# CrystalAnalyst/Lsm

Measured on AMD Instinct MI355X. Metric: GiB/s device-resident SSTable block encode+decode, 4 KiB blocks, 1/2/4/8 GPU, higher is better.
Workload: dtype u8; 1 GPU; U: 1048576 blocks/GPU x block_size 4096, decode + re-encode (16-B uniform keys, 100-B values); blocks_per_gpu=1048576, entries_per_gpu=32474205, encoded_bytes_per_gpu=4226189427, decoded_bytes_per_gpu=4286595060, block_size=4096, segments_per_gpu=2045, parallelism=block-sharded x1 (no data-path collective), encode_output=segments packed (lsmblk_encode_batch), rccl_world=1

## Files before the change

lsm_amd/csrc/lsmblk_gpu.hip:

```cpp
#include "lsmblk_dev.hpp"

namespace {


struct DecodeArgs {
  const uint8_t* blocks;
  const uint64_t* blk_off;
  uint64_t nblk;
  uint8_t* keys;
  uint32_t* key_off;
  uint8_t* vals;
  uint32_t* val_off;
  uint64_t* ts;
  uint64_t entry_cap, key_cap, val_cap;
  uint64_t* stats;
  const uint32_t* agg;
  const uint64_t* tile_pre;
  uint32_t tail;
  uint64_t* blk_ent;
  uint32_t skip;
  uint64_t* bagg;
  uint64_t* bbase;
  uint64_t* tagg;
  uint64_t* tinc;
  uint64_t lag;
  uint64_t lag_bytes;
  uint64_t* dbg;
  uint32_t tag, poll;
};

constexpr uint32_t kTile = 64;
constexpr uint32_t kDbgTiles = 32768, kDbgWords = 16 + 8 * kDbgTiles;
__device__ __forceinline__ void dbg_trace(uint64_t* dbg, uint64_t t, uint32_t k) {
  if (kDiag && dbg && t < kDbgTiles && lane_id() == 0) dbg[16 + 8 * t + k] = __builtin_amdgcn_s_memrealtime();
}


constexpr uint32_t kLB = 2;
constexpr uint32_t kDecMB = 2;
#ifndef LSMBLK_XEB
#define LSMBLK_XEB 4
#endif
constexpr uint32_t kEB = LSMBLK_XEB;
constexpr uint32_t kEBBlock = 2;


constexpr uint32_t kDecImg = 4128;
constexpr uint32_t kDecMaxE = 128;
constexpr uint32_t kDecKeyImg = 2176;
constexpr uint32_t kDecMapN = 256;
constexpr uint32_t kDecOut = 4032;
static_assert(kDecOut <= 16 * kDecMapN && 16 * kDecMapN <= kDecImg, "the chunk map covers the value run");

struct alignas(16) DecLds {
  uint8_t img[kDecImg];
  alignas(16) uint8_t kimg[kDecKeyImg];
  alignas(16) uint16_t cmap[kDecMapN];
};
static_assert(sizeof(DecLds) <= (160 << 10) / 24, "decode LDS: room for 24 blocks per CU");

struct DecTables {
  uint16_t epos[kDecMaxE], pfx[kDecMaxE], sfx[kDecMaxE];
  uint32_t kout[kDecMaxE + 1], vout[kDecMaxE + 1];
};
static_assert(sizeof(DecTables) <= kDecImg, "large-block tables overlay the image");

struct DecEnt {
  uint32_t epos, p, s, kout, vout, vl;
};

__device__ __forceinline__ void lds_read16(const uint8_t* base, uint32_t x, uint32_t (&v)[4]) {
  const u32x4 q = *reinterpret_cast<const u32x4*>(base + x);
  v[0] = q.x, v[1] = q.y, v[2] = q.z, v[3] = q.w;
}

constexpr int kLdAux = 0;

template <class Img>
__device__ void dec_simple_outputs(const DecodeArgs& a, const Img& im, const BlockHdr& h,
                                   uint64_t E0, uint64_t K0, uint64_t V0) {
  const uint32_t l = lane_id();
  uint64_t kc = 0, vc = 0;
  for (uint32_t c = 0; c < h.n; c += 64) {
    const uint32_t k = c + l;
    uint32_t off = 0, p = 0, s = 0, vl = 0;
    if (k < h.n) parse_entry(im, h, k, off, p, s, vl);
    const uint64_t kl = p + s;
    const uint64_t ki = wave_incl_scan<uint64_t>(kl), vi = wave_incl_scan<uint64_t>(vl);
    const uint64_t kpos = K0 + kc + ki - kl, vpos = V0 + vc + vi - vl;
    kc += __shfl(ki, 63, 64);
    vc += __shfl(vi, 63, 64);
    if (k < h.n) {
      const uint64_t e = E0 + k;
      if (e < a.entry_cap) {
        a.ts[e] = im.u64(off + 4 + s);
        a.key_off[e] = uint32_t(kpos);
        a.val_off[e] = uint32_t(vpos);
      }
      for (uint32_t t = 0; t < p; ++t)
        if (kpos + t < a.key_cap) a.keys[kpos + t] = uint8_t(im.u8(4 + t));
      for (uint32_t t = 0; t < s; ++t)
        if (kpos + p + t < a.key_cap) a.keys[kpos + p + t] = uint8_t(im.u8(off + 4 + t));
      for (uint32_t t = 0; t < vl; ++t)
        if (vpos + t < a.val_cap) a.vals[vpos + t] = uint8_t(im.u8(off + 14 + s + t));
    }
  }
}

__device__ __forceinline__ void st16(const rsrc_t& R, uint32_t off, const uint32_t (&v)[4]) {
  const u32x4 q = {v[0], v[1], v[2], v[3]};
  __builtin_amdgcn_raw_buffer_store_b128(q, R, off, 0, 0);
}

__device__ __forceinline__ void st_short(const rsrc_t& R, uint32_t off, uint32_t len, const uint32_t (&v)[4]) {
  if (len >= 8) {
    __builtin_amdgcn_raw_buffer_store_b64(u32x2{v[0], v[1]}, R, off, 0, 0);
    const uint32_t x = len - 8, sh = x & 3;
    const uint32_t w0 = x < 4 ? v[0] : v[1], w1 = x < 4 ? v[1] : v[2], w2 = x < 4 ? v[2] : v[3];
    __builtin_amdgcn_raw_buffer_store_b64(
        u32x2{__builtin_amdgcn_alignbyte(w1, w0, sh), __builtin_amdgcn_alignbyte(w2, w1, sh)}, R, off + x, 0, 0);
  } else if (len >= 4) {
    __builtin_amdgcn_raw_buffer_store_b32(v[0], R, off, 0, 0);
    __builtin_amdgcn_raw_buffer_store_b32(__builtin_amdgcn_alignbyte(v[1], v[0], len - 4), R, off + len - 4, 0, 0);
  } else {
    for (uint32_t i = 0; i < len; ++i)
      __builtin_amdgcn_raw_buffer_store_b8(uint8_t(v[0] >> (8 * i)), R, off + i, 0, 0);
  }
}

__device__ __forceinline__ void lds_st_short(uint8_t* p, uint32_t len, const uint32_t (&v)[4]) {
  if (len >= 8) {
    const uint32_t x = len - 8, sh = x & 3;
    const uint32_t w0 = x < 4 ? v[0] : v[1], w1 = x < 4 ? v[1] : v[2], w2 = x < 4 ? v[2] : v[3];
    *reinterpret_cast<u32x2*>(p) = u32x2{v[0], v[1]};
    *reinterpret_cast<u32x2*>(p + x) = u32x2{__builtin_amdgcn_alignbyte(w1, w0, sh), __builtin_amdgcn_alignbyte(w2, w1, sh)};
  } else if (len >= 4) {
    *reinterpret_cast<uint32_t*>(p) = v[0];
    *reinterpret_cast<uint32_t*>(p + len - 4) = __builtin_amdgcn_alignbyte(v[1], v[0], len - 4);
  } else {
    for (uint32_t i = 0; i < len; ++i) p[i] = uint8_t(v[0] >> (8 * i));
  }
}

struct GlbSink {
  rsrc_t RK, RV;
  uint32_t kb, vb;
  __device__ __forceinline__ void put16(bool val, uint32_t off, const uint32_t (&v)[4]) const {
    st16(val ? RV : RK, (val ? vb : kb) + off, v);
  }
  __device__ __forceinline__ void put_short(bool val, uint32_t off, uint32_t len, const uint32_t (&v)[4]) const {
    st_short(val ? RV : RK, (val ? vb : kb) + off, len, v);
  }
};
struct LdsSink {
  uint8_t* kimg;
  uint32_t kb;
  uint16_t* cmap;
  uint32_t vb;
  __device__ __forceinline__ void put16(bool, uint32_t off, const uint32_t (&v)[4]) const {
    *reinterpret_cast<u32x4*>(kimg + kb + off) = u32x4{v[0], v[1], v[2], v[3]};
  }
  __device__ __forceinline__ void put_short(bool, uint32_t off, uint32_t len, const uint32_t (&v)[4]) const {
    lds_st_short(kimg + kb + off, len, v);
  }
};

template <class Sink>
__device__ __forceinline__ void dec_entry_runs(const DecodeArgs& a, DecLds& L, uint32_t lead, uint32_t n,
                                               const DecEnt (&ent)[2], uint64_t E0, uint64_t K0, uint64_t V0,
                                               const Sink& out, uint32_t skip, uint32_t (&eh)[2][4],
                                               uint32_t (&et)[2][4]) {
  const uint32_t l = lane_id();
  const uint8_t* img = L.img;
  const uint32_t fk = lead + 4;
#pragma unroll
  for (uint32_t it = 0; it < 2; ++it) {
    if (64 * it >= n) break;
    const uint32_t k = 64 * it + l;
    const bool live = k < n;
    const uint32_t epos = ent[it].epos, p = ent[it].p, s = ent[it].s;
    const uint32_t kout = ent[it].kout, vout = ent[it].vout, vl = ent[it].vl;
    const uint32_t sb = lead + epos + 4;
    const uint32_t kl = p + s;
    const bool kirr = live && (kl < 16 || sb < p);
    const bool kuni = !__ballot(kirr);
    const uint32_t nkmax = __builtin_amdgcn_readlane(wave_incl_max32(live ? (kl + 15) >> 4 : 0u), 63);
    uint32_t nvmax = 0;
    if constexpr (!std::is_same_v<Sink, LdsSink>)
      nvmax = __builtin_amdgcn_readlane(wave_incl_max32(live && vl >= 16 ? (vl + 15) >> 4 : 0u), 63);
    if (!live) continue;
    if (!(skip & 8)) {
      const uint64_t e = E0 + k;
      const u32x2 q = LSMBLK_XALIGNED_LDS ? lds_qw_al(img, sb + s) : *reinterpret_cast<const u32x2*>(img + sb + s);
      a.ts[e] = __builtin_bswap64((uint64_t(q.y) << 32) | q.x);
      a.key_off[e] = uint32_t(K0 + kout);
      a.val_off[e] = uint32_t(V0 + vout);
    }
    if (!(skip & 2)) {
      auto merged = [&](uint32_t o, uint32_t (&v)[4]) {
        const u32x4 sq = *reinterpret_cast<const u32x4*>(img + sb + o - p);
        const u32x4 fq = *reinterpret_cast<const u32x4*>(img + fk + o);
        const uint32_t sv[4] = {sq.x, sq.y, sq.z, sq.w}, fv[4] = {fq.x, fq.y, fq.z, fq.w};
#pragma unroll
        for (uint32_t d = 0; d < 4; ++d) {
          const int32_t nf = int32_t(p) - int32_t(o + 4 * d);
          const uint32_t m = nf <= 0 ? 0u : nf >= 4 ? ~0u : (1u << (8 * nf)) - 1;
          v[d] = (fv[d] & m) | (sv[d] & ~m);
        }
      };
      if (kuni) {
        for (uint32_t t = 0; t < nkmax; ++t) {
          const uint32_t o = min(16 * t, kl - 16);
          uint32_t v[4];
          merged(o, v);
          out.put16(false, kout + o, v);
        }
      } else {
        for (uint32_t t = 0; t < kl; t += 16) {
          const uint32_t o = kl >= 16 ? min(t, kl - 16) : 0u;
          uint32_t v[4];
          if (sb + o >= p) {
            merged(o, v);
          } else {
#pragma unroll
            for (uint32_t d = 0; d < 4; ++d) {
              uint32_t wd = 0;
              for (uint32_t i = 0; i < 4; ++i) {
                const uint32_t x = o + 4 * d + i;
                wd |= uint32_t(x < p ? img[fk + x] : img[sb + x - p]) << (8 * i);
              }
              v[d] = wd;
            }
          }
          if (kl >= 16) out.put16(false, kout + o, v);
          else out.put_short(false, kout, kl, v);
        }
      }
    }
    const uint32_t src = sb + s + 10;
    if constexpr (std::is_same_v<Sink, LdsSink>) {
      if (vl && !(skip & 4)) {
        lds_read16(img, src, eh[it]);
        lds_read16(img, src + (vl > 16 ? vl - 16 : 0u), et[it]);
        const uint32_t vD = out.vb + vout;
        const uint32_t d = src - vD;
        for (uint32_t c = (vD + 15) >> 4; 16 * c + 16 <= vD + vl; ++c) out.cmap[c] = uint16_t(d + 16 * c);
      }
    } else if (!(skip & 4)) {
      if (vl >= 16) {
        for (uint32_t i0 = 0; i0 < nvmax; i0 += kLB) {
          u32x4 q[kLB];
          uint32_t o[kLB];
          const uint32_t am = (skip & 32) ? 15u : (skip & 64) ? 3u : 0u;
#pragma unroll
          for (uint32_t j = 0; j < kLB; ++j) {
            o[j] = min(16 * (i0 + j), vl - 16);
            q[j] = *reinterpret_cast<const u32x4*>(img + ((src + o[j]) & ~am));
          }
#pragma unroll
          for (uint32_t j = 0; j < kLB; ++j) {
            const uint32_t v[4] = {q[j].x, q[j].y, q[j].z, q[j].w};
            const uint32_t xa = (out.vb + vout + o[j]) & ~am;
            out.put16(true, xa >= out.vb ? xa - out.vb : xa + am + 1 - out.vb, v);
          }
        }
      } else if (vl) {
        const u32x4 q = *reinterpret_cast<const u32x4*>(img + src);
        const uint32_t v[4] = {q.x, q.y, q.z, q.w};
        out.put_short(true, vout, vl, v);
      }
    }
  }
}

template <uint32_t B = kLB>
__device__ __forceinline__ void flush_run(uint8_t* gdst_aligned, const uint8_t* lds, uint32_t lo, uint32_t len) {
  flush_chunks<B, LSMBLK_XDEC_STORE>(gdst_aligned, lds, lo, len, lane_id(), 64);
}

template <uint32_t B>
__device__ __forceinline__ void flush_run_masked(uint8_t* gdst_aligned, const uint8_t* lds, uint32_t lo, uint32_t len) {
  const uint32_t end = lo + len, nc = (end + 15) >> 4;
  const uint32_t l = lane_id();
  for (uint32_t c0 = 0; c0 < nc; c0 += 64 * B) {
    u32x4 q[B];
#pragma unroll
    for (uint32_t j = 0; j < B; ++j) {
      const uint32_t c = c0 + 64 * j + l;
      if (c < nc) q[j] = *reinterpret_cast<const u32x4*>(lds + 16 * c);
    }
#pragma unroll
    for (uint32_t j = 0; j < B; ++j) {
      const uint32_t c = c0 + 64 * j + l;
      if (c < nc) {
        const uint32_t v[4] = {q[j].x, q[j].y, q[j].z, q[j].w};
        const uint32_t a0 = 16 * c < lo ? lo - 16 * c : 0u;
        const uint32_t a1 = min(end - 16 * c, 16u);
        store_chunk(gdst_aligned + 16 * c, v, a0, a1);
      }
    }
  }
}

__device__ void dec_fast_outputs(const DecodeArgs& a, DecLds& L, uint32_t lead, const BlockHdr& h,
                                 const DecEnt (&ent)[2], uint64_t E0, uint64_t K0, uint64_t V0, uint32_t K,
                                 uint32_t V, uint32_t skip) {
  const uint32_t l = lane_id();
  const uint32_t n = h.n;
  const uint32_t kb = uint32_t(K0 & 15), vb = uint32_t(V0 & 15);
  int32_t dprev = 0;
  bool mono = true;
#pragma unroll
  for (uint32_t it = 0; it < 2; ++it) {
    if (64 * it >= n) break;
    const bool live = 64 * it + l < n;
    const int32_t d = live ? int32_t(lead + ent[it].epos + 14 + ent[it].s) - int32_t(vb + ent[it].vout) : 0x7FFFFFFF;
    const int32_t up = __shfl_up(d, 1, 64);
    mono = mono && d >= (l ? up : dprev);
    dprev = __builtin_amdgcn_readlane(d, 63);
  }
  const uint32_t krun = (kb + K + 15) & ~15u;
  if (!__ballot(!mono) && krun <= kDecKeyImg && krun + ((vb + V + 15) & ~15u) <= kDecOut) {
    static_assert(sizeof(DecLds::cmap) == 32 * 16, "the map is zeroed by 32 lanes");
    if (l < 32) reinterpret_cast<u32x4*>(L.cmap)[l] = u32x4{0, 0, 0, 0};
    wave_sync();
    uint32_t eh[2][4] = {}, et[2][4] = {};
    dec_entry_runs(a, L, lead, n, ent, E0, K0, V0, LdsSink{L.kimg, kb, L.cmap, vb}, skip, eh, et);
    wave_sync();
    flush_run(a.keys + (K0 - kb), L.kimg, kb, K);
    if (!(skip & 4)) {
      const uint32_t nw = (vb + V) >> 4;
      for (uint32_t c0 = 0; c0 < nw; c0 += 64 * kDecMB) {
        uint32_t src[kDecMB] = {};
        u32x4 v[kDecMB] = {};
#pragma unroll
        for (uint32_t j = 0; j < kDecMB; ++j) {
          const uint32_t c = c0 + 64 * j + l;
          src[j] = c < nw ? L.cmap[c] : 0u;
        }
#pragma unroll
        for (uint32_t j = 0; j < kDecMB; ++j)
          if (src[j]) v[j] = *reinterpret_cast<const u32x4*>(L.img + src[j]);
#pragma unroll
        for (uint32_t j = 0; j < kDecMB; ++j)
          if (src[j]) *reinterpret_cast<u32x4*>(L.img + 16 * (c0 + 64 * j + l)) = v[j];
      }
      wave_sync();
#pragma unroll
      for (uint32_t it = 0; it < 2; ++it) {
        if (64 * it >= n) break;
        const uint32_t vl = ent[it].vl;
        uint8_t* const o = L.img + vb + ent[it].vout;
        if (64 * it + l >= n) continue;
        if (vl >= 16) {
          *reinterpret_cast<u32x4*>(o) = u32x4{eh[it][0], eh[it][1], eh[it][2], eh[it][3]};
          *reinterpret_cast<u32x4*>(o + vl - 16) = u32x4{et[it][0], et[it][1], et[it][2], et[it][3]};
        } else if (vl) {
          lds_st_short(o, vl, eh[it]);
        }
      }
      wave_sync();
      flush_run(a.vals + (V0 - vb), L.img, vb, V);
    }
  } else {
    const GlbSink g{make_rsrc_exact(a.keys + (K0 - kb), kb + K), make_rsrc_exact(a.vals + (V0 - vb), vb + V), kb, vb};
    uint32_t eh[2][4], et[2][4];
    dec_entry_runs(a, L, lead, n, ent, E0, K0, V0, g, skip, eh, et);
  }
}

constexpr uint32_t kBigB = 8;

__device__ __forceinline__ u32x4 gload16(const rsrc_t& R, uint32_t off) {
  return __builtin_amdgcn_raw_buffer_load_b128(R, off, 0, 0);
}

__device__ __forceinline__ void copy_run(const rsrc_t& RS, uint32_t so, uint32_t lim, const rsrc_t& RD, uint32_t dof,
                                         uint32_t len) {
  if (len == 0) return;
  if (len < 16) {
    uint32_t v[4] = {0, 0, 0, 0};
    if (so + 16 <= lim) {
      const u32x4 q = gload16(RS, so);
      v[0] = q.x, v[1] = q.y, v[2] = q.z, v[3] = q.w;
    } else {
      for (uint32_t i = 0; i < len; ++i) v[i >> 2] |= __builtin_amdgcn_raw_buffer_load_b8(RS, so + i, 0, 0) << (8 * (i & 3));
    }
    st_short(RD, dof, len, v);
    return;
  }
  const uint32_t np = (len + 15) >> 4, last = len - 16;
  for (uint32_t j0 = 0; j0 < np; j0 += kBigB) {
    u32x4 q[kBigB];
#pragma unroll
    for (uint32_t j = 0; j < kBigB; ++j)
      if (j0 + j < np) q[j] = gload16(RS, so + min(16 * (j0 + j), last));
#pragma unroll
    for (uint32_t j = 0; j < kBigB; ++j)
      if (j0 + j < np) {
        const uint32_t v[4] = {q[j].x, q[j].y, q[j].z, q[j].w};
        st16(RD, dof + min(16 * (j0 + j), last), v);
      }
  }
}

__device__ __forceinline__ void copy_run1(const rsrc_t& RS, uint32_t so, uint32_t lim, const rsrc_t& RD, uint32_t dof,
                                          uint32_t len) {
  if (len < 16) {
    copy_run(RS, so, lim, RD, dof, len);
    return;
  }
  const uint32_t last = len - 16;
  for (uint32_t o = 0;; o += 16) {
    const uint32_t x = min(o, last);
    const u32x4 q = gload16(RS, so + x);
    const uint32_t v[4] = {q.x, q.y, q.z, q.w};
    st16(RD, dof + x, v);
    if (x == last) break;
  }
}

constexpr uint32_t kCoop = 16;
__device__ __forceinline__ void copy_run_wave(const rsrc_t& RS, uint32_t so, const rsrc_t& RD, uint32_t dof,
                                              uint32_t len) {
  const uint32_t l = lane_id();
  const uint32_t np = (len + 15) >> 4, last = len - 16;
  for (uint32_t j0 = 0; j0 < np; j0 += 64 * kBigB) {
    u32x4 q[kBigB];
#pragma unroll
    for (uint32_t j = 0; j < kBigB; ++j) {
      const uint32_t idx = j0 + 64 * j + l;
      if (idx < np) q[j] = gload16(RS, so + min(16 * idx, last));
    }
#pragma unroll
    for (uint32_t j = 0; j < kBigB; ++j) {
      const uint32_t idx = j0 + 64 * j + l;
      if (idx < np) {
        const uint32_t v[4] = {q[j].x, q[j].y, q[j].z, q[j].w};
        st16(RD, dof + min(16 * idx, last), v);
      }
    }
  }
}

constexpr uint32_t kCopyScratch = 4 * 64 + 64;
static_assert(4 * kCopyScratch <= kDecKeyImg, "the decode's large-block path lends its key image");

template <uint32_t B>
struct CopyBatch {
  u32x4 q[B];
  uint32_t dst[B];
};

template <uint32_t B, bool PIN = false>
__device__ __forceinline__ void copy_issue(const rsrc_t& RS, uint32_t g0, uint32_t total, uint32_t np, uint32_t first,
                                           uint32_t* sc, uint32_t& carry, CopyBatch<B>& c) {
  const uint32_t l = lane_id();
  if constexpr (PIN) {
#pragma unroll
    for (uint32_t j = 0; j < B; ++j) asm volatile("" : "=v"(c.q[j]));
  }
  const u32x4* rec = reinterpret_cast<const u32x4*>(sc);
  uint32_t* mark = sc + 4 * 64;
  uint32_t own[B];
#pragma unroll
  for (uint32_t j = 0; j < B; ++j) {
    const uint32_t G = g0 + 64 * j;
    own[j] = 0;
    if (G < total) {
      mark[l] = 0;
      wave_sync();
      if (np != 0 && first - G < 64u) mark[first - G] = l + 1;
      wave_sync();
      const uint32_t m = max(wave_incl_max32(mark[l]), carry);
      carry = __builtin_amdgcn_readlane(m, 63);
      own[j] = m - 1;
      wave_sync();
    }
  }
#pragma unroll
  for (uint32_t j = 0; j < B; ++j) {
    const uint32_t g = g0 + 64 * j + l;
    c.dst[j] = ~0u;
    if (g < total) {
      const u32x4 r = rec[own[j]];
      const uint32_t off = min(16 * (g - r.w), r.z);
      const uint32_t src = r.x + off;
      if constexpr (PIN) {
        if (j == 0) asm volatile("s_nop 4\n\tbuffer_load_dwordx4 %0, %1, %2, 0 offen" : "+v"(c.q[j]) : "v"(src), "s"(RS));
        else asm volatile("buffer_load_dwordx4 %0, %1, %2, 0 offen" : "+v"(c.q[j]) : "v"(src), "s"(RS));
      } else {
        c.q[j] = gload16(RS, src);
      }
      c.dst[j] = r.y + off;
    }
  }
}

template <uint32_t B>
__device__ __forceinline__ void copy_land(CopyBatch<B>& c) {
  asm volatile("s_waitcnt vmcnt(0)" ::: "memory");
#pragma unroll
  for (uint32_t j = 0; j < B; ++j) asm volatile("" : "+v"(c.q[j]));
}

template <uint32_t B>
__device__ __forceinline__ void copy_store(const rsrc_t& RD, const CopyBatch<B>& c) {
#pragma unroll
  for (uint32_t j = 0; j < B; ++j)
    if (c.dst[j] != ~0u) {
      const uint32_t v[4] = {c.q[j].x, c.q[j].y, c.q[j].z, c.q[j].w};
      st16(RD, c.dst[j], v);
    }
}

struct NoAfter {
  __device__ void operator()(uint32_t, uint32_t, uint32_t) const {}
};
template <uint32_t B = kBigB, bool PIN = false, class After = NoAfter>
__device__ __forceinline__ void copy_long_runs(bool longrun, const rsrc_t& RS, uint32_t so, const rsrc_t& RD,
                                               uint32_t dof, uint32_t len, uint32_t* sc, const After& after = After()) {
  const uint32_t l = lane_id();
  const uint32_t np = longrun ? (len + 15) >> 4 : 0u;
  const uint32_t incl = wave_incl_scan32(np);
  const uint32_t total = __builtin_amdgcn_readlane(incl, 63);
  const uint32_t first = incl - np;
  if (total == 0) {
    after(first, 0u, ~0u);
    return;
  }
  wave_sync();
  reinterpret_cast<u32x4*>(sc)[l] = u32x4{so, dof, len - 16, first};
  uint32_t carry = 0;
  for (uint32_t g0 = 0; g0 < total; g0 += 64 * B) {
    CopyBatch<B> c;
    copy_issue<B, PIN>(RS, g0, total, np, first, sc, carry, c);
    if constexpr (PIN) copy_land(c);
    copy_store(RD, c);
    after(first, g0, g0 + 64 * B >= total ? ~0u : g0 + 64 * B);
  }
}

__device__ __forceinline__ void dec_big_entry(const DecodeArgs& a, const DecTables& L, const GlbImg& im, uint32_t k,
                                              uint32_t lim, const rsrc_t& RK, uint32_t kb, uint64_t E0, uint64_t K0,
                                              uint64_t V0) {
  const rsrc_t& R = im.r;
  const uint32_t lead = im.lead, fk = lead + 4;
  const uint32_t epos = L.epos[k], p = L.pfx[k], s = L.sfx[k], kout = L.kout[k];
  const uint32_t sb = lead + epos + 4, kl = p + s;
  const uint64_t e = E0 + k;
  a.ts[e] = im.u64(epos + 4 + s);
  a.key_off[e] = uint32_t(K0 + kout);
  a.val_off[e] = uint32_t(V0 + L.vout[k]);
  for (uint32_t t = 0; t < kl; t += 16) {
    const uint32_t o = kl >= 16 ? min(t, kl - 16) : 0u;
    uint32_t v[4];
    if (sb + o >= p && sb + o - p + 16 <= lim && fk + o + 16 <= lim) {
      const u32x4 sq = gload16(R, sb + o - p), fq = gload16(R, fk + o);
      const uint32_t sv[4] = {sq.x, sq.y, sq.z, sq.w}, fv[4] = {fq.x, fq.y, fq.z, fq.w};
#pragma unroll
      for (uint32_t d = 0; d < 4; ++d) {
        const int32_t nf = int32_t(p) - int32_t(o + 4 * d);
        const uint32_t m = nf <= 0 ? 0u : nf >= 4 ? ~0u : (1u << (8 * nf)) - 1;
        v[d] = (fv[d] & m) | (sv[d] & ~m);
      }
    } else {
#pragma unroll
      for (uint32_t d = 0; d < 4; ++d) {
        uint32_t wd = 0;
        for (uint32_t i = 0; i < 4; ++i) {
          const uint32_t x = o + 4 * d + i;
          wd |= (x < p ? im.u8(4 + x) : im.u8(epos + 4 + x - p)) << (8 * i);
        }
        v[d] = wd;
      }
    }
    if (kl >= 16) st16(RK, kb + kout + o, v);
    else st_short(RK, kb + kout, kl, v);
  }
}

#ifndef LSMBLK_XDBB
#define LSMBLK_XDBB 8
#endif
constexpr uint32_t kDecBigB = LSMBLK_XDBB;

__device__ void dec_big_outputs(const DecodeArgs& a, const DecTables& L, const rsrc_t& R, uint32_t lead,
                                const BlockHdr& h, uint32_t n, uint64_t Eb, uint64_t K0, uint64_t V0, uint32_t K,
                                uint32_t V, uint32_t* sc) {
  const uint32_t l = lane_id();
  const uint32_t kb = uint32_t(K0 & 15), vb = uint32_t(V0 & 15);
  const rsrc_t RK = make_rsrc_exact(a.keys + (K0 - kb), kb + K), RV = make_rsrc_exact(a.vals + (V0 - vb), vb + V);
  const GlbImg im{R, lead};
  const uint32_t lim = lead + h.len;
  for (uint32_t c = 0; c < n; c += 64) {
    const uint32_t k = c + l;
    const bool live = k < n;
    uint32_t vsrc = 0, vdst = 0, vl = 0;
    if (live) {
      dec_big_entry(a, L, im, k, lim, RK, kb, Eb, K0, V0);
      vsrc = lead + L.epos[k] + 14 + L.sfx[k];
      vdst = vb + L.vout[k];
      vl = L.vout[k + 1] - L.vout[k];
      if (vl < kCoop) copy_run(R, vsrc, lim, RV, vdst, vl);
    }
    copy_long_runs<kDecBigB, true>(live && vl >= kCoop, R, vsrc, RV, vdst, vl, sc);
  }
}

template <bool lagm, class Mid, class Post, class PreWait>
__device__ void decode_block(const DecodeArgs& a, DecLds& L, uint64_t b, uint64_t start, uint64_t end, Mid&& mid,
                             Post&& post, PreWait&& pre_wait) {
  const uint32_t l = lane_id();
  uint32_t err = 0;
  const uint64_t tb = b / kTile, jb = b % kTile;
  uint32_t cn = 0, ck = 0, cv = 0;
  uint64_t tp0 = 0, tp1 = 0, tp2 = 0, gb = 0;
  if constexpr (!lagm) {
    if (l < jb) {
      const uint64_t q = tb * kTile + l;
      cn = a.agg[3 * q];
      ck = a.agg[3 * q + 1];
      cv = a.agg[3 * q + 2];
    }
    tp0 = a.tile_pre[3 * tb], tp1 = a.tile_pre[3 * tb + 1], tp2 = a.tile_pre[3 * tb + 2];
  }
  uint32_t len = 0;
  if (end < start + a.tail || end - start > 0x7FFFFFF0ull) err |= LSMBLK_ERR_MALFORMED;
  else len = uint32_t(end - start) - a.tail;
  const uint8_t* bp = a.blocks + start;
  const uint32_t lead = uni(uint32_t(reinterpret_cast<uintptr_t>(bp) & 15));
  const uint8_t* abase = bp - lead;
  const rsrc_t R = make_rsrc(abase, lead + len);
  const bool fits = lead + len + 15 <= kDecImg;

  BlockHdr h;
  if (fits) {
    const uint32_t nchunk = (lead + len + 15) >> 4;
    u32x4 v[5];
    if constexpr (lagm) {
      const uint32_t o = 16 * l, o4 = o + 4096;
      asm volatile(
          "s_nop 4\n\t"
          "buffer_load_dwordx4 %0, %5, %7, 0 offen\n\t"
          "buffer_load_dwordx4 %1, %5, %7, 0 offen offset:1024\n\t"
          "buffer_load_dwordx4 %2, %5, %7, 0 offen offset:2048\n\t"
          "buffer_load_dwordx4 %3, %5, %7, 0 offen offset:3072\n\t"
          "buffer_load_dwordx4 %4, %6, %7, 0 offen"
          : "=&v"(v[0]), "=&v"(v[1]), "=&v"(v[2]), "=&v"(v[3]), "=&v"(v[4])
          : "v"(o), "v"(o4), "s"(R));
      mid();
      asm volatile("s_waitcnt vmcnt(0)" ::: "memory");
#pragma unroll
      for (uint32_t i = 0; i < 5; ++i) asm volatile("" : "+v"(v[i]));
    } else {
#pragma unroll
      for (uint32_t i = 0; i < 5; ++i)
        v[i] = __builtin_amdgcn_raw_buffer_load_b128(R, (l + 64 * i) * 16, 0, kLdAux);
    }
#pragma unroll
    for (uint32_t i = 0; i < 5; ++i)
      if (l + 64 * i < nchunk) *reinterpret_cast<u32x4*>(L.img + (l + 64 * i) * 16) = v[i];
    wave_sync();
    post();
    if (lagm && l < 3 && !(diag_mask(a.skip) & 4096)) gb = gload(a.bbase + 3 * b + l, 0);
// ... 3455 lines not shown
```

Before: 1048 GiB/s.

## Gather decoded value chunks straight to global memory via slot map, skipping LDS compaction

The LDS-staged value decode used to compact 16-byte chunks inside the image, patch entry heads and tails back in, then flush the whole run to global memory. It now writes the partial head and tail chunks of each entry into separate slots in the key image, tagged with a slot marker in the chunk map. The gather loop then reads each chunk from the image or a slot and stores it straight to global memory, with byte stores only for the run's partial first and last chunks. This removes one LDS write pass, two wave barriers and the separate flush, at the cost of a wave scan and more map bookkeeping.

Result: no change. 1055 GiB/s (median of 6 runs) (+0.7%).

```diff
diff --git a/lsm_amd/csrc/lsmblk_gpu.hip b/lsm_amd/csrc/lsmblk_gpu.hip
--- a/lsm_amd/csrc/lsmblk_gpu.hip
+++ b/lsm_amd/csrc/lsmblk_gpu.hip
@@ -49,6 +49,8 @@
 constexpr uint32_t kDecMaxE = 128;
 constexpr uint32_t kDecKeyImg = 2176;
 constexpr uint32_t kDecMapN = 256;
+constexpr uint32_t kDecSlot = 0x8000;
+static_assert(kDecImg < kDecSlot, "a source byte in the image is below the slot marker");
 constexpr uint32_t kDecOut = 4032;
 static_assert(kDecOut <= 16 * kDecMapN && 16 * kDecMapN <= kDecImg, "the chunk map covers the value run");
 
@@ -240,9 +242,10 @@
     const uint32_t src = sb + s + 10;
     if constexpr (std::is_same_v<Sink, LdsSink>) {
       if (vl && !(skip & 4)) {
+        const uint32_t vD = out.vb + vout;
+        const uint32_t tl = (vD + vl) & 15;
         lds_read16(img, src, eh[it]);
-        lds_read16(img, src + (vl > 16 ? vl - 16 : 0u), et[it]);
-        const uint32_t vD = out.vb + vout;
+        lds_read16(img, src + (vl > tl ? vl - tl : 0u), et[it]);
         const uint32_t d = src - vD;
         for (uint32_t c = (vD + 15) >> 4; 16 * c + 16 <= vD + vl; ++c) out.cmap[c] = uint16_t(d + 16 * c);
       }
@@ -329,38 +332,58 @@
     wave_sync();
     flush_run(a.keys + (K0 - kb), L.kimg, kb, K);
     if (!(skip & 4)) {
-      const uint32_t nw = (vb + V) >> 4;
-      for (uint32_t c0 = 0; c0 < nw; c0 += 64 * kDecMB) {
-        uint32_t src[kDecMB] = {};
+      const uint32_t end = vb + V, nc = (end + 15) >> 4;
+      const bool head_part = vb != 0 || end < 16, tail_part = (end & 15) != 0;
+      const uint32_t cf = head_part ? 1u : 0u, ce = tail_part ? nc - 1 : nc;
+      uint8_t* const gv = a.vals + (V0 - vb);
+      wave_sync();
+      static_assert(16 * (kDecMaxE + 1) <= kDecKeyImg, "the key image holds the shared chunks");
+      uint32_t mbase = 0;
+#pragma unroll
+      for (uint32_t it = 0; it < 2; ++it) {
+        if (64 * it >= n) break;
+        const bool live = 64 * it + l < n;
+        const uint32_t vl = live ? ent[it].vl : 0u;
+        const uint32_t S = vb + ent[it].vout, E = S + vl;
+        const uint32_t ch = S >> 4, ct = (E - 1) >> 4;
+        const uint32_t m = vl && (E >> 4) > ((S + 15) >> 4) ? (E >> 4) - ((S + 15) >> 4) : 0u;
+        const uint32_t mi = wave_incl_scan32(m);
+        const uint32_t mb = mbase + mi - m;
+        mbase += __builtin_amdgcn_readlane(mi, 63);
+        if (!vl) continue;
+        const uint32_t ao = S & 15, tl = E & 15;
+        const uint32_t hl = ch == ct ? (vl == 16 ? 0u : vl) : (ao ? 16 - ao : 0u);
+        if (hl) {
+          lds_st_short(L.kimg + 16 * (ch - mb) + ao, hl, eh[it]);
+          L.cmap[ch] = uint16_t(kDecSlot | (ch - mb));
+        }
+        if (ch != ct && tl) {
+          lds_st_short(L.kimg + 16 * (ct - mb - m), tl, et[it]);
+          L.cmap[ct] = uint16_t(kDecSlot | (ct - mb - m));
+        }
+      }
+      wave_sync();
+      {
+        const uint32_t x = l < 16 ? l : 16 * (nc - 1) + (l - 16);
+        const uint32_t sx = l < 16 ? l : 16 * (nc - 1 - mbase) + (l - 16);
+        if (l < 32 && (l < 16 ? head_part : tail_part) && x >= vb && x < end) gv[x] = L.kimg[sx];
+      }
+      for (uint32_t c0 = cf; c0 < ce; c0 += 64 * kDecMB) {
         u32x4 v[kDecMB] = {};
+        uint32_t src[kDecMB];
 #pragma unroll
         for (uint32_t j = 0; j < kDecMB; ++j) {
           const uint32_t c = c0 + 64 * j + l;
-          src[j] = c < nw ? L.cmap[c] : 0u;
+          src[j] = c < ce ? L.cmap[c] : 0u;
         }
 #pragma unroll
         for (uint32_t j = 0; j < kDecMB; ++j)
-          if (src[j]) v[j] = *reinterpret_cast<const u32x4*>(L.img + src[j]);
+          if (c0 + 64 * j + l < ce)
+            v[j] = *reinterpret_cast<const u32x4*>(src[j] & kDecSlot ? L.kimg + 16 * (src[j] & (kDecSlot - 1)) : L.img + src[j]);
 #pragma unroll
         for (uint32_t j = 0; j < kDecMB; ++j)
-          if (src[j]) *reinterpret_cast<u32x4*>(L.img + 16 * (c0 + 64 * j + l)) = v[j];
-      }
-      wave_sync();
-#pragma unroll
-      for (uint32_t it = 0; it < 2; ++it) {
-        if (64 * it >= n) break;
-        const uint32_t vl = ent[it].vl;
-        uint8_t* const o = L.img + vb + ent[it].vout;
-        if (64 * it + l >= n) continue;
-        if (vl >= 16) {
-          *reinterpret_cast<u32x4*>(o) = u32x4{eh[it][0], eh[it][1], eh[it][2], eh[it][3]};
-          *reinterpret_cast<u32x4*>(o + vl - 16) = u32x4{et[it][0], et[it][1], et[it][2], et[it][3]};
-        } else if (vl) {
-          lds_st_short(o, vl, eh[it]);
-        }
-      }
-      wave_sync();
-      flush_run(a.vals + (V0 - vb), L.img, vb, V);
+          if (c0 + 64 * j + l < ce) st_chunk16<LSMBLK_XDEC_STORE>(gv + 16 * (c0 + 64 * j + l), v[j]);
+      }
     }
   } else {
     const GlbSink g{make_rsrc_exact(a.keys + (K0 - kb), kb + K), make_rsrc_exact(a.vals + (V0 - vb), vb + V), kb, vb};
```
